# prime-slam/octreelib

Hardware: AMD Instinct MI355X
Metric: Mpoints/s insert+subdivide+RANSAC (higher is better)
Workload: dtype f64; 1 GPU; BASELINE config 3: Grid 1 m voxels, 10000000 planar points per GPU (scene 32x32x32 voxels), insert + subdivide(len>64) + map_leaf_points_cuda_ransac(H=1024, k=6, thr=0.01, poses_per_batch=10) incl. apply_mask; points_per_gpu=10000000, K=64, hypotheses=1024, leaves=575543

## Files before the change

### octreelib_amd/csrc/ransac.hip

```cpp
#include <algorithm>
#include <cstdlib>
#include <type_traits>

#include "forest.h"
#include "lookback.h"
#include "wave_utils.h"

namespace {

__device__ __forceinline__ double div_by_small_int(double c, int k) {
  const double kd = (double)k;
  const double zh = 1.0 / kd;
  const double zl = fma(-kd, zh, 1.0) / kd;
  const double a = fabs(c);
  if (!((int(a > 1e-290) | int(c == 0.0)) & int(a < 1e290))) return c / kd;
  return copysign(fma(c, zh, c * zl), c);
}

__device__ __forceinline__ bool coord_in_fast_range(double v) {
  const uint32_t hi = (uint32_t)__double2hiint(v), lo = (uint32_t)__double2loint(v);
  const uint32_t e = (hi >> 20) & 0x7FFu;
  return (e - (1023u - 30u)) <= 60u || (hi | lo) == 0u;
}

__device__ __forceinline__ void div3_by_small_int(double& cx, double& cy, double& cz, int k, bool fast = false) {
  const double kd = (double)k;
  const double zh = 1.0 / kd;
  const double zl = fma(-kd, zh, 1.0) / kd;
  if (fast) {
    cx = fma(cx, zh, cx * zl);
    cy = fma(cy, zh, cy * zl);
    cz = fma(cz, zh, cz * zl);
    return;
  }
  const double ax = fabs(cx), ay = fabs(cy), az = fabs(cz);
  const int ok = (int(ax > 1e-290) | int(cx == 0.0)) & int(ax < 1e290) &
                 (int(ay > 1e-290) | int(cy == 0.0)) & int(ay < 1e290) &
                 (int(az > 1e-290) | int(cz == 0.0)) & int(az < 1e290);
  if (!ok) {
    cx /= kd;
    cy /= kd;
    cz /= kd;
    return;
  }
  cx = copysign(fma(cx, zh, cx * zl), cx);
  cy = copysign(fma(cy, zh, cy * zl), cy);
  cz = copysign(fma(cz, zh, cz * zl), cz);
}

__device__ __forceinline__ double sqrt_rn_inrange(double s) {
  const double y = __builtin_amdgcn_rsq(s);
  double g = s * y;
  double h = y * 0.5;
  const double r = fma(-h, g, 0.5);
  g = fma(g, r, g);
  h = fma(h, r, h);
  double d = fma(-g, g, s);
  g = fma(d, h, g);
  d = fma(-g, g, s);
  return fma(d, h, g);
}
__device__ __forceinline__ double sqrt_rn_guarded(double s) {
  if (!(int(s >= 0x1p-700) & int(s < 0x1p1000))) return __dsqrt_rn(s);
  return sqrt_rn_inrange(s);
}

__device__ __forceinline__ void div3_by_norm_inrange(double& ax, double& ay, double& az, double norm) {
  double r = __builtin_amdgcn_rcp(norm);
  double e = fma(-norm, r, 1.0);
  r = fma(r, e, r);
  e = fma(-norm, r, 1.0);
  r = fma(r, e, r);
  const double qx = ax * r, qy = ay * r, qz = az * r;
  ax = copysign(fma(fma(-norm, qx, ax), r, qx), ax);
  ay = copysign(fma(fma(-norm, qy, ay), r, qy), ay);
  az = copysign(fma(fma(-norm, qz, az), r, qz), az);
}
__device__ __forceinline__ void div3_by_norm(double& ax, double& ay, double& az, double norm) {
  const double lo = 0x1p-400, hi = 0x1p500;
  const int ok = int(norm >= lo) & int(norm < hi) & (int(fabs(ax) >= lo) | int(ax == 0.0)) &
                 (int(fabs(ay) >= lo) | int(ay == 0.0)) & (int(fabs(az) >= lo) | int(az == 0.0));
  if (!ok) {
    ax /= norm;
    ay /= norm;
    az /= norm;
    return;
  }
  div3_by_norm_inrange(ax, ay, az, norm);
}

__device__ __forceinline__ void plane_from_moments(double cx, double cy, double cz, double xx, double xy,
                                                   double xz, double yy, double yz, double zz,
                                                   float (&plane)[4], bool fast = false) {
  const double det_x = yy * zz - yz * yz;
  const double det_y = xx * zz - xz * xz;
  const double det_z = xx * yy - xy * xy;
  const double cA = xz * yz - xy * zz;
  const double cB = xy * yz - xz * yy;
  const double cC = xy * xz - yz * xx;
  const bool is_x = det_x > det_y && det_x > det_z;
  const bool is_y = !is_x && det_y > det_z;
  double ax = is_x ? det_x : (is_y ? cA : cB);
  double ay = is_x ? cA : (is_y ? det_y : cC);
  double az = is_x ? cB : (is_y ? cC : det_z);
  const double s = ax * ax + ay * ay + az * az;
  if (fast && (uint32_t)__double2hiint(s) >= ((1023u - 400u) << 20)) {
    const double norm = sqrt_rn_inrange(s);
    div3_by_norm_inrange(ax, ay, az, norm);
  } else {
    const double norm = sqrt_rn_guarded(s);
    if (norm == 0.0) {
      plane[0] = plane[1] = plane[2] = plane[3] = 0.0f;
      return;
    }
    div3_by_norm(ax, ay, az, norm);
  }
  const double d = -(ax * cx + ay * cy + az * cz);
  plane[0] = (float)ax;
  plane[1] = (float)ay;
  plane[2] = (float)az;
  plane[3] = (float)d;
}

template <int KT, int KMAX>
__device__ __forceinline__ void plane_from_samples(const double (&sx)[KMAX],
                                                   const double (&sy)[KMAX],
                                                   const double (&sz)[KMAX], int k_rt,
                                                   float (&plane)[4], bool fast = false) {
  const int k = KT > 0 ? KT : k_rt;
  double cx = 0.0, cy = 0.0, cz = 0.0;
  if (fast) {
    cx = sx[0];
    cy = sy[0];
    cz = sz[0];
  } else {
    asm volatile("" ::: "memory");
    cx += sx[0];
    cy += sy[0];
    cz += sz[0];
  }
#pragma unroll
  for (int i = 1; i < (KT > 0 ? KT : KMAX); ++i) {
    if (i < k) {
      cx += sx[i];
      cy += sy[i];
      cz += sz[i];
    }
  }
  div3_by_small_int(cx, cy, cz, k, fast);
  double xx = 0.0, xy = 0.0, xz = 0.0, yy = 0.0, yz = 0.0, zz = 0.0;
#pragma unroll
  for (int i = 0; i < (KT > 0 ? KT : KMAX); ++i) {
    if (i < k) {
      const double rx = sx[i] - cx;
      const double ry = sy[i] - cy;
      const double rz = sz[i] - cz;
      if (i == 0) {
        xx = rx * rx;
// ... 56 lines not shown
  *risky = (x - (double)g0) > (1.0 - 0x1p-20);
  return g0 < n ? g0 : n;
}

__device__ __forceinline__ void plane_streamed(const double* __restrict__ hyp_row, int k, const BlockDesc& d,
                                               const double* __restrict__ xyz, float (&plane)[4]) {
  auto point = [&](int i) {
    const int g = sample_index_exact(hyp_row[i], d.n, d.vstart);
    return (g < d.n) ? (int64_t)d.pstart + g : (int64_t)d.pspill;
  };
  double cx = 0.0, cy = 0.0, cz = 0.0;
  for (int i = 0; i < k; ++i) {
    const int64_t p = point(i);
    cx += xyz[3 * p];
    cy += xyz[3 * p + 1];
    cz += xyz[3 * p + 2];
  }
  const double kd = (double)k;
  cx = cx / kd;
  cy = cy / kd;
  cz = cz / kd;
  double xx = 0.0, xy = 0.0, xz = 0.0, yy = 0.0, yz = 0.0, zz = 0.0;
  for (int i = 0; i < k; ++i) {
    const int64_t p = point(i);
    const double rx = xyz[3 * p] - cx, ry = xyz[3 * p + 1] - cy, rz = xyz[3 * p + 2] - cz;
    xx += rx * rx;
    xy += rx * ry;
    xz += rx * rz;
    yy += ry * ry;
    yz += ry * rz;
    zz += rz * rz;
  }
  plane_from_moments(cx, cy, cz, xx, xy, xz, yy, yz, zz, plane);
}

template <int THREADS, int HPL, int KT>
__device__ __forceinline__ void ransac_block_global(const BlockDesc& d, int be,
                                                    const double* __restrict__ xyz,
                                                    const double* __restrict__ hyp, int H, int k_rt,
                                                    double thr, const RansacOut& out,
                                                    unsigned long long* s_best, float* s_plane) {
  constexpr int KS = KT > 0 ? KT : RS_KMAX;
  const int k = KT > 0 ? KT : k_rt;
  const int n = d.n;
  const int64_t pstart = d.pstart;
  const double* __restrict__ pts = xyz + 3 * pstart;
  double pa[HPL], pb[HPL], pc[HPL], pd[HPL];
  int cnt[HPL];
#pragma unroll
  for (int q = 0; q < HPL; ++q) {
    const int t = threadIdx.x + q * THREADS;
    cnt[q] = -1;
    pa[q] = pb[q] = pc[q] = pd[q] = 0.0;
    if (t < H) {
      float pf[4];
      if constexpr (KT < 0) {
        plane_streamed(hyp + (int64_t)t * k, k, d, xyz, pf);
      } else {
        double sx[KS], sy[KS], sz[KS];
#pragma unroll
        for (int i = 0; i < KS; ++i) {
          sx[i] = sy[i] = sz[i] = 0.0;
          if (i < k) {
            const int g = sample_index_exact(hyp[(int64_t)t * k + i], n, d.vstart);
            const int64_t p = (g < n) ? pstart + g : (int64_t)d.pspill;
            sx[i] = xyz[3 * p];
            sy[i] = xyz[3 * p + 1];
            sz[i] = xyz[3 * p + 2];
          }
        }
        plane_from_samples<KT, KS>(sx, sy, sz, k, pf);
      }
      pa[q] = (double)pf[0];
      pb[q] = (double)pf[1];
      pc[q] = (double)pf[2];
      pd[q] = (double)pf[3];
      cnt[q] = 0;
    }
    __builtin_amdgcn_sched_barrier(0);
  }
  for (int i = 0; i < n; ++i) {
    const double x = pts[3 * (int64_t)i], y = pts[3 * (int64_t)i + 1], z = pts[3 * (int64_t)i + 2];
#pragma unroll
    for (int q = 0; q < HPL; ++q)
      cnt[q] += (plane_distance(pa[q], pb[q], pc[q], pd[q], x, y, z) < thr) ? 1 : 0;
  }
  unsigned long long best = 0;
#pragma unroll
  for (int q = 0; q < HPL; ++q) {
    const int t = threadIdx.x + q * THREADS;
    if (t < H) {
      const unsigned long long key =
          ((unsigned long long)(unsigned)cnt[q] << 32) | (unsigned)(0x7FFFFFFF - t);
      best = key > best ? key : best;
    }
  }
#pragma unroll
  for (int off = 32; off > 0; off >>= 1) {
    const unsigned long long o = __shfl_xor(best, off);
    best = o > best ? o : best;
  }
  if ((threadIdx.x & 63) == 0) s_best[threadIdx.x >> 6] = best;
  __syncthreads();
  best = s_best[0];
#pragma unroll
  for (int w = 1; w < THREADS / 64; ++w) best = s_best[w] > best ? s_best[w] : best;
  const int win = 0x7FFFFFFF - (int)(unsigned)(best & 0xFFFFFFFFu);
#pragma unroll
  for (int q = 0; q < HPL; ++q) {
    if ((int)threadIdx.x + q * THREADS == win) {
      const float f0 = (float)pa[q], f1 = (float)pb[q], f2 = (float)pc[q], f3 = (float)pd[q];
      s_plane[0] = f0; s_plane[1] = f1; s_plane[2] = f2; s_plane[3] = f3;
      if (out.plane) {
        out.plane[4 * (int64_t)be + 0] = f0; out.plane[4 * (int64_t)be + 1] = f1;
        out.plane[4 * (int64_t)be + 2] = f2; out.plane[4 * (int64_t)be + 3] = f3;
      }
      if (out.count) out.count[be] = cnt[q];
      if (out.index) out.index[be] = win;
    }
  }
  __syncthreads();
  const double a = (double)s_plane[0], bb = (double)s_plane[1], c = (double)s_plane[2],
               dd = (double)s_plane[3];
  for (int i = threadIdx.x; i < n; i += THREADS)
    out.mask[pstart + i] = (plane_distance(a, bb, c, dd, pts[3 * (int64_t)i], pts[3 * (int64_t)i + 1],
                                           pts[3 * (int64_t)i + 2]) < thr) ? 1 : 0;
}

typedef float f4 __attribute__((ext_vector_type(4)));
__device__ __forceinline__ float fma32(float a, float b, float c) { return __builtin_fmaf(a, b, c); }
__device__ __forceinline__ float min3abs(float m, float a, float b) {
  float r;
  asm("v_min3_f32 %0, %1, |%2|, |%3|" : "=v"(r) : "v"(m), "v"(a), "v"(b));
  return r;
}

template <int CTRL, int ROW_MASK>
__device__ __forceinline__ uint32_t dpp_u32(uint32_t v) {
  return (uint32_t)__builtin_amdgcn_update_dpp((int)v, (int)v, CTRL, ROW_MASK, 0xF, false);
}
__device__ __forceinline__ uint32_t wave_max_u32(uint32_t v) {
  v = max(v, dpp_u32<0xB1, 0xF>(v));
  v = max(v, dpp_u32<0x4E, 0xF>(v));
  v = max(v, dpp_u32<0x141, 0xF>(v));
  v = max(v, dpp_u32<0x140, 0xF>(v));
  v = max(v, dpp_u32<0x142, 0xA>(v));
  v = max(v, dpp_u32<0x143, 0xC>(v));
  return (uint32_t)__builtin_amdgcn_readlane((int)v, 63);
}
__device__ __forceinline__ float wave_max_nonneg_f32(float m) {
  return __uint_as_float(wave_max_u32(__float_as_uint(m)));
}

template <int THREADS>
__device__ __forceinline__ void stage_local(unsigned tx, double ox, double oy, double oz, const BlockDesc& d,
                                            double px, double py, double pz, f4* loc,
                                            float* wext, uint32_t* wfast, float* ext_out = nullptr,
                                            uint32_t* fast_out = nullptr) {
  float m = 0.f;
  if ((int)tx < d.n) {
    const float u = (float)(px - ox), v = (float)(py - oy), w = (float)(pz - oz);
    loc[tx] = f4{u, v, w, 0.f};
    m = fmaxf(fabsf(u), fmaxf(fabsf(v), fabsf(w)));
    if (!(m == m) || u != u || v != v || w != w) m = __int_as_float(0x7f800000);
  }
  m = wave_max_nonneg_f32(m);
  const bool inr = coord_in_fast_range(px) && coord_in_fast_range(py) && coord_in_fast_range(pz);
  const bool wave_fast = __all(inr);
  if (ext_out) {
    *ext_out = m;
    *fast_out = wave_fast ? 1u : 0u;
  } else if ((tx & 63) == 0) {
    wext[tx >> 6] = m;
    wfast[tx >> 6] = wave_fast ? 1u : 0u;
  }
}

template <int NH>
__device__ __forceinline__ void screen_group(const f4* __restrict__ loc, int n, const float* fa,
                                             const float* fb, const float* fc, const float* sto,
                                             float nthr2, int* cnt, float* margin) {
  float mg[2][NH];
#pragma unroll
  for (int h = 0; h < NH; ++h) mg[0][h] = mg[1][h] = __int_as_float(0x7f800000);
  for (int base = 0; base < n; base += 32) {
    const int m = __builtin_amdgcn_readfirstlane(min(32, n - base));
    uint32_t hist[NH];
#pragma unroll
    for (int h = 0; h < NH; ++h) hist[h] = 0;
    auto score = [&](const f4 L, float (&e)[NH]) {
#pragma unroll
      for (int h = 0; h < NH; ++h) {
        const float sv = fma32(fa[h], L.x, fma32(fb[h], L.y, fma32(fc[h], L.z, sto[h])));
        e[h] = fma32(sv, sv, nthr2);
        hist[h] = __builtin_amdgcn_alignbit(hist[h], __float_as_uint(e[h]), 31);
      }
    };
    int i = 0;
    for (; i + 4 <= m; i += 4) {
      const f4 L0 = loc[base + i], L1 = loc[base + i + 1], L2 = loc[base + i + 2],
               L3 = loc[base + i + 3];
      float e0[NH], e1[NH], e2[NH], e3[NH];
      score(L0, e0);
      score(L1, e1);
      score(L2, e2);
      score(L3, e3);
#pragma unroll
      for (int h = 0; h < NH; ++h) {
        mg[0][h] = min3abs(mg[0][h], e0[h], e1[h]);
        mg[1][h] = min3abs(mg[1][h], e2[h], e3[h]);
      }
    }
    for (; i < m; ++i) {
      float e[NH];
      score(loc[base + i], e);
#pragma unroll
      for (int h = 0; h < NH; ++h) mg[0][h] = min3abs(mg[0][h], e[h], e[h]);
    }
#pragma unroll
    for (int h = 0; h < NH; ++h) cnt[h] += __popc(hist[h]);
  }
#pragma unroll
  for (int h = 0; h < NH; ++h) margin[h] = fminf(mg[0][h], mg[1][h]);
}

struct PreConst {
  float qa, qb, qc;
  float e35;
  float thrblk;
};
__device__ __forceinline__ bool prescreen_constants(float extent, double ox, double oy, double oz, double thr,
                                                    PreConst& pc) {
  const float up = 0x1.004p0f;
  const float u = 0x1p-24f;
  const float E = extent;
  const float G = ((float)(fabs(ox) + fabs(oy) + fabs(oz)) + E) * 0x1.0002p0f;
  const float k1 = 16.f * (12.f * u + 0x1p-46f * (G / E) * 0x1.0002p0f) * 0x1.0002p0f;
  const float k0 = 16.f * (3.f * u * (E * E) + 0x1p-46f * G * E) * 0x1.0002p0f;
  pc.qa = (k1 + 0x1p-20f + k1 * k1 * 0x1p-4f) * up;
  pc.qb = (k0 + k1 * k0 * 0x1p-3f) * up;
  pc.qc = (k0 * k0 * 0x1p-4f) * up + 0x1p-98f;
  pc.e35 = 3.5f * E * up;
  const float eblk = (64.f * u * E + 0x1p-21f * G) * 0x1.0002p0f;
  const float thr_f = (float)thr * 0x1.0002p0f;
  pc.thrblk = (thr_f + eblk) * up;
  return E >= 0x1p-7f && E <= 0x1p7f && thr >= 0x1p-40 && thr <= 0x1p40 && eblk * 8.f <= thr_f;
}

template <int NH>
__device__ __forceinline__ void screen_ub(const f4* __restrict__ loc, int n, const float* fa, const float* fb,
                                          const float* fc, const float* sto, const float* T2, int* cnt) {
  for (int base = 0; base < n; base += 32) {
    const int m = __builtin_amdgcn_readfirstlane(min(32, n - base));
    uint32_t hist[NH];
#pragma unroll
    for (int h = 0; h < NH; ++h) hist[h] = 0;
    auto score = [&](const f4 L) {
#pragma unroll
      for (int h = 0; h < NH; ++h) {
        const float sv = fma32(fa[h], L.x, fma32(fb[h], L.y, fma32(fc[h], L.z, sto[h])));
        const float e = fma32(sv, sv, -T2[h]);
        hist[h] = __builtin_amdgcn_alignbit(hist[h], __float_as_uint(e), 31);
      }
    };
    int i = 0;
    for (; i + 4 <= m; i += 4) {
      const f4 L0 = loc[base + i], L1 = loc[base + i + 1], L2 = loc[base + i + 2], L3 = loc[base + i + 3];
      score(L0);
      score(L1);
      score(L2);
      score(L3);
    }
    for (; i < m; ++i) score(loc[base + i]);
#pragma unroll
    for (int h = 0; h < NH; ++h) cnt[h] += __popc(hist[h]);
  }
}

#ifdef RS_COUNTS
constexpr int RS_NSTAMPS = 24;
__device__ unsigned long long g_rs_stamps[RS_NSTAMPS];
#define RS_COUNT_INIT unsigned long long _rs_acc[RS_NSTAMPS] = {0, 0, 0, 0, 0, 0, 0, 0, 0, 0, 0, 0, 0, 0, 0, 0,  \
                                                                0, 0, 0, 0, 0, 0, 0, 0};                             \
                      const unsigned long long _rs_m0 = __builtin_amdgcn_s_memtime(),                      \
                                               _rs_r0 = __builtin_amdgcn_s_memrealtime()
#define RS_COUNT(k, v) _rs_acc[k] += (unsigned long long)(v)
#define RS_COUNT_FLUSH                                                                  \
  do {                                                                                  \
    if (threadIdx.x == 0) {                                                             \
      _rs_acc[0] = __builtin_amdgcn_s_memtime() - _rs_m0;                               \
      _rs_acc[1] = __builtin_amdgcn_s_memrealtime() - _rs_r0;                           \
      _rs_acc[10] += 1;                                                                 \
      for (int _k = 0; _k < RS_NSTAMPS; ++_k) atomicAdd(&g_rs_stamps[_k], _rs_acc[_k]); \
    }                                                                                   \
  } while (0)
#else
#define RS_COUNT_INIT do {} while (0)
#define RS_COUNT(k, v) do {} while (0)
#define RS_COUNT_FLUSH do {} while (0)
#endif

template <int THREADS, int HPL, int KT, bool FULLH, bool PT>
__global__ __launch_bounds__(THREADS, rs_minwaves(THREADS, KT)) void k_ransac(
    const double* __restrict__ xyz, const BlockDesc* __restrict__ sdesc,
    const uint32_t* __restrict__ lo_ptr, const uint32_t* __restrict__ hi_ptr, const double* __restrict__ hyp, int H,
    int k_rt, double thr, RansacOut out, const uint2* __restrict__ pos_tab, int no_prescreen) {
  static_assert(!PT || (KT > 0 && KT <= 6), "the position table packs up to six positions and their risk bits");
  static_assert(THREADS * HPL <= 1024, "hypothesis index in 10 bits");
  constexpr bool PRE = PT && KT >= 3 && HPL >= 2;
  constexpr int W = THREADS / 64;
  constexpr bool PARK = PRE && W == 1;
  constexpr int KS = KT > 0 ? KT : RS_KMAX;
  constexpr int GW = (KS + 3) / 4;
  constexpr int PRE_LIST = THREADS == 64 ? 512 : 256;
  constexpr bool OWN_LIST = PRE && W > 1;
  __shared__ uint16_t s_surv_all[OWN_LIST ? W : 1][OWN_LIST ? PRE_LIST : 1];
  uint16_t* const s_surv_own = s_surv_all[OWN_LIST ? (threadIdx.x >> 6) : 0];
  const int k = KT > 0 ? KT : k_rt;
  __shared__ double s_pts[3][3][THREADS];
  __shared__ uint32_t s_wbest[2][W];
  __shared__ float s_wplane[2][W][4];
  __shared__ f4 s_loc[3][THREADS];
  static_assert(!(PRE && W == 1) || PRE_LIST * sizeof(uint16_t) <= sizeof(s_loc[0]), "the survivor list fits an s_loc buffer");
  __shared__ float s_wext[3][W];
  __shared__ uint32_t s_wfast[3][W];
  const int lo = lo_ptr ? (int)*lo_ptr : 0;
  const int hi = (int)*hi_ptr;
  const int nbs = hi - lo;
  const int C = (nbs + (int)gridDim.x - 1) / (int)gridDim.x;
  int j = lo + (int)blockIdx.x * C;
  const int j_end = min(hi, j + C);
  if (j >= j_end) return;
  float ext_carry = 0.f;
  uint32_t fast_carry = 0;
  BlockDesc cur = sdesc[j];
  BlockDesc nxt = cur;
  if (j + 1 < j_end) nxt = sdesc[j + 1];
  {
    double px = 0.0, py = 0.0, pz = 0.0;
    if ((int)threadIdx.x <= cur.n) {
      const int64_t p = ((int)threadIdx.x < cur.n) ? (int64_t)cur.pstart + threadIdx.x : (int64_t)cur.pspill;
      px = xyz[3 * p];
      py = xyz[3 * p + 1];
      pz = xyz[3 * p + 2];
      s_pts[0][0][threadIdx.x] = px;
      s_pts[0][1][threadIdx.x] = py;
      s_pts[0][2][threadIdx.x] = pz;
    }
    stage_local<THREADS>(threadIdx.x, xyz[3 * (int64_t)cur.pstart], xyz[3 * (int64_t)cur.pstart + 1],
                         xyz[3 * (int64_t)cur.pstart + 2], cur, px, py, pz, s_loc[0], s_wext[0], s_wfast[0],
                         W == 1 ? &ext_carry : nullptr, W == 1 ? &fast_carry : nullptr);
  }
  __syncthreads();
  int buf = 0, par = 0;
  RS_COUNT_INIT;
  for (;;) {
    unsigned tx = threadIdx.x;
    asm volatile("" : "+v"(tx));
    const bool has_next = j + 1 < j_end;
    BlockDesc nxt2 = nxt;
    if (j + 2 < j_end) nxt2 = sdesc[j + 2];
    double rx = 0.0, ry = 0.0, rz = 0.0;
    auto pre_here = [&]() {
      unsigned t = tx;
      if constexpr (PARK) asm volatile("" : "+v"(t));
      return has_next && (int)t <= nxt.n;
    };
    const int nbuf = buf == 2 ? 0 : buf + 1;
    uint16_t* const s_surv = PARK ? (uint16_t*)&s_loc[nbuf][0] : s_surv_own;
    auto prefetch = [&]() {
      if (pre_here()) {
        const int64_t p = ((int)tx < nxt.n) ? (int64_t)nxt.pstart + tx : (int64_t)nxt.pspill;
        rx = xyz[3 * p];
        ry = xyz[3 * p + 1];
        rz = xyz[3 * p + 2];
      }
    };
    auto park = [&]() {
      if (pre_here()) {
        s_pts[nbuf][0][tx] = rx;
        s_pts[nbuf][1][tx] = ry;
        s_pts[nbuf][2][tx] = rz;
      }
    };
    double nox = 0.0, noy = 0.0, noz = 0.0;
    if constexpr (!PARK) {
      prefetch();
      if (has_next) {
        nox = xyz[3 * (int64_t)nxt.pstart];
        noy = xyz[3 * (int64_t)nxt.pstart + 1];
        noz = xyz[3 * (int64_t)nxt.pstart + 2];
      }
    }
    const int n = cur.n;
    const int be = (int)cur.pad[1];
    const double* __restrict__ lx = s_pts[buf][0];
    const double* __restrict__ ly = s_pts[buf][1];
    const double* __restrict__ lz = s_pts[buf][2];

    RS_COUNT(8, 1);
    RS_COUNT(11, n);
    float extent = W == 1 ? ext_carry : s_wext[buf][0];
#pragma unroll
    for (int w = 1; w < W; ++w) extent = fmaxf(extent, s_wext[buf][w]);
    uint32_t fastw = W == 1 ? fast_carry : s_wfast[buf][0];
#pragma unroll
    for (int w = 1; w < W; ++w) fastw &= s_wfast[buf][w];
    const bool blk_fast = __builtin_amdgcn_readfirstlane((int)fastw) != 0;
    const bool blk_sane = thr >= 0x1p-40 && thr <= 0x1p40 && extent < 0x1p60f;
    const bool fast_screen = blk_fast && thr >= 0x1p-40 && thr <= 0x1p40;
    const f4* __restrict__ loc = s_loc[buf];
    struct BlkConst {
      double ox, oy, oz;
      double delta_blk, dprime_thr, thr2;
      float nthr2;
      float delta_blk_f, thr2_f, dprime_thr_f;
    };
    auto blk_consts = [&]() {
      double th = thr;
      if constexpr (PARK) asm volatile("" : "+s"(th));
      BlkConst c;
      c.ox = lx[0]; c.oy = ly[0]; c.oz = lz[0];
      c.delta_blk = fma(0x1p-23 * 9.0, (double)extent,
                        0x1p-49 * (fabs(c.ox) + fabs(c.oy) + fabs(c.oz) + (double)extent + 1.0));
      c.dprime_thr = 0x1p-21 * (th * th);
      c.thr2 = th + th;
      c.nthr2 = -(float)(th * th);
      c.delta_blk_f = (float)c.delta_blk * 0x1.0002p0f;
      c.thr2_f = (float)(th + th) * 0x1.0002p0f;
      c.dprime_thr_f = (float)c.dprime_thr * 0x1.0002p0f;
      return c;
    };
    const BlkConst bc0 = blk_consts();
    auto consts_here = [&]() {
      if constexpr (PARK) return blk_consts();
      else return bc0;
    };
    const double ox = bc0.ox, oy = bc0.oy, oz = bc0.oz;

    uint32_t gpk[GW], rk = 0;
    float fa = 0.f, fb = 0.f, fc = 0.f, fd = 0.f, sto = 0.f, sdl = 0.f;
    int cnt = 0;
    auto load_pos = [&](const int t, const bool act) {
#pragma unroll
      for (int w = 0; w < GW; ++w) gpk[w] = 0;
      rk = 0;
      if constexpr (PT) {
        const uint2 e = pos_tab[(size_t)n * (size_t)H + (size_t)(act ? t : 0)];
        gpk[0] = e.x;
        if (GW > 1) gpk[GW - 1] = e.y & 0xFFFFu;
        rk = e.y >> 16;
      } else if (act) {
        const double* __restrict__ row = hyp + (int64_t)t * k;
#pragma unroll
        for (int i = 0; i < KS; ++i) {
          if (i < k) {
            bool risky;
            const int g = sample_index_cached(row[i], n, &risky);
            gpk[i >> 2] |= (uint32_t)g << (8 * (i & 3));
            rk |= (risky || g == n) ? (1u << i) : 0u;
          }
        }
      }
    };
    auto fit = [&](const int t, const bool act) {
      cnt = 0;
      fa = fb = fc = fd = sto = sdl = 0.f;
      if (FULLH || act) {
        const BlkConst bc = consts_here();
        const double ox = bc.ox, oy = bc.oy, oz = bc.oz, delta_blk = bc.delta_blk, dprime_thr = bc.dprime_thr;
        const float delta_blk_f = bc.delta_blk_f, thr2_f = bc.thr2_f, dprime_thr_f = bc.dprime_thr_f;
        double sx[KS], sy[KS], sz[KS];
        if (!__any(rk != 0u)) {
#pragma unroll
          for (int i = 0; i < KS; ++i) {
            sx[i] = sy[i] = sz[i] = 0.0;
            if (i < k) {
              const int g = (int)((gpk[i >> 2] >> (8 * (i & 3))) & 0xFFu);
              sx[i] = lx[g];
              sy[i] = ly[g];
              sz[i] = lz[g];
            }
          }
        } else {
#pragma unroll
          for (int i = 0; i < KS; ++i) {
            sx[i] = sy[i] = sz[i] = 0.0;
            if (i < k) {
              int g = (int)((gpk[i >> 2] >> (8 * (i & 3))) & 0xFFu);
              if (rk & (1u << i)) g = sample_index_exact(hyp[(int64_t)t * k + i], n, cur.vstart);
              sx[i] = lx[g];
              sy[i] = ly[g];
              sz[i] = lz[g];
            }
          }
        }
        float pf[4];
        plane_from_samples<KT, KS>(sx, sy, sz, k, pf, blk_fast);
        const double A = (double)pf[0], B = (double)pf[1], Cc = (double)pf[2], D = (double)pf[3];
        const double to = fma(A, ox, fma(B, oy, fma(Cc, oz, D)));
        fa = pf[0]; fb = pf[1]; fc = pf[2]; fd = pf[3];
        sto = (float)to;
        if (fast_screen) {
          const float dl = fma32(fabsf(sto), 0x1.0002p-21f, fma32(fabsf(pf[3]), 0x1.0002p-49f, delta_blk_f));
          sdl = fma32(dl, thr2_f + dl, dprime_thr_f) * 0x1.0002p0f;
        } else {
          const double delta = fma(0x1p-21, fabs(to), fma(0x1p-49, fabs(D), delta_blk));
          const double dprime = fma(delta, bc.thr2 + delta, dprime_thr) * 1.000001;
          const bool sane = blk_sane && (fabs(to) < 0x1p60);
          sdl = sane ? (float)dprime : __int_as_float(0x7f800000);
        }
      }
    };
    auto score = [&](const bool act) {
      float margin[1];
      int c1[1] = {0};
      RS_COUNT(14, 1);
      RS_COUNT(15, n);
      screen_group<1>(loc, n, &fa, &fb, &fc, &sto, consts_here().nthr2, c1, margin);
      cnt = c1[0];
      const bool redo = act && !(margin[0] > sdl);
      unsigned long long todo = __ballot(redo);
      RS_COUNT(13, __popcll(todo));
      while (todo) {
        const int src = __ffsll((long long)todo) - 1;
        todo &= todo - 1;
        const double A = (double)__uint_as_float(__builtin_amdgcn_readlane(__float_as_uint(fa), src));
        const double B = (double)__uint_as_float(__builtin_amdgcn_readlane(__float_as_uint(fb), src));
        const double Cc = (double)__uint_as_float(__builtin_amdgcn_readlane(__float_as_uint(fc), src));
        const double D = (double)__uint_as_float(__builtin_amdgcn_readlane(__float_as_uint(fd), src));
        int c = 0;
        for (int base = 0; base < n; base += 64) {
          const int ii = base + (int)(tx & 63u);
          const bool in = ii < n && plane_distance(A, B, Cc, D, lx[ii < n ? ii : 0], ly[ii < n ? ii : 0],
                                                   lz[ii < n ? ii : 0]) < thr;
          c += __popcll(__ballot(in));
        }
        if ((int)(tx & 63u) == src) cnt = c;
      }
    };
    uint32_t best = 0;
    float wa = 0.f, wb = 0.f, wc = 0.f, wd = 0.f;
    auto take = [&](const int t, const bool act) {
      if (act) {
        const uint32_t key = ((uint32_t)(cnt + 1) << 10) | (uint32_t)(1023 - t);
        if (key > best) {
          best = key;
          wa = fa; wb = fb; wc = fc; wd = fd;
        }
      }
    };
    {
      const int t = (int)tx;
      const bool act = FULLH || t < H;
      load_pos(t, act);
      fit(t, act);
      if constexpr (PARK) prefetch();
      score(act);
      take(t, act);
    }
    if constexpr (HPL > 1) {
      int Lcur = (int)wave_max_u32((FULLH || (int)tx < H) ? (uint32_t)cnt : 0u);
      if (Lcur != n) {
        int S = 0;
        bool use_list = false;
        if constexpr (PRE) {
          PreConst pc;
          const bool elig = prescreen_constants(extent, ox, oy, oz, thr, pc) && blk_fast && !no_prescreen;
          if (elig) {
            RS_COUNT(4, 1);
            constexpr bool TWO = THREADS == 64;
            typedef uint32_t __attribute__((may_alias)) u32a;
            const int budget = n - Lcur;
            int m1 = n, qhead = 0, qtail = 0;
            bool two_stage = false;
            f4* ploc = nullptr;
            u32a *qlo = nullptr, *qhi = nullptr;
            if constexpr (TWO) {
              m1 = min(n, (budget + RS_STAGE1_SLACK + 3) & ~3);
              two_stage = n - m1 >= RS_STAGE2_MIN;
              if (two_stage) {
                const int third = buf == 0 ? 2 : buf - 1;
                ploc = s_loc[third];
                qlo = (u32a*)&s_pts[third][0][0];
                qhi = (u32a*)&s_pts[buf == 2 ? 0 : buf + 1][0][0];
                static_assert(3 * RS_STAGE2_RING * sizeof(uint32_t) <= sizeof(s_pts[0]), "three words per idle buffer");
                const unsigned long long wl = __ballot(cnt == Lcur);
                const int src = __ffsll((long long)wl) - 1;
                const float A = __uint_as_float(__builtin_amdgcn_readlane(__float_as_uint(fa), src));
                const float B = __uint_as_float(__builtin_amdgcn_readlane(__float_as_uint(fb), src));
                const float Cc = __uint_as_float(__builtin_amdgcn_readlane(__float_as_uint(fc), src));
                const float To = __uint_as_float(__builtin_amdgcn_readlane(__float_as_uint(sto), src));
                const bool mine = (int)tx < n;
                const f4 Lp = loc[mine ? tx : 0];
                const float sv = fma32(A, Lp.x, fma32(B, Lp.y, fma32(Cc, Lp.z, To)));
                const bool far = mine && !(fma32(sv, sv, consts_here().nthr2) < 0.f);
                const unsigned long long mf = __ballot(far), mn = __ballot(mine && !far);
                const unsigned long long mm = far ? mf : mn;
                const int pos = (far ? 0 : __popcll(mf)) +
                                (int)__builtin_amdgcn_mbcnt_hi((uint32_t)(mm >> 32), __builtin_amdgcn_mbcnt_lo((uint32_t)mm, 0u));
                if (mine) ploc[pos] = Lp;
                __builtin_amdgcn_fence(__ATOMIC_ACQ_REL, "wavefront");
              } else {
                RS_COUNT(19, 1);
              }
            }
            auto survive = [&](const bool sv, const uint32_t ub, const int t) {
              const unsigned long long mk = __ballot(sv);
              if (sv) {
                const int pos = S + (int)__builtin_amdgcn_mbcnt_hi((uint32_t)(mk >> 32), __builtin_amdgcn_mbcnt_lo((uint32_t)mk, 0u));
                if (pos < PRE_LIST) s_surv[pos] = (uint16_t)((ub << 10) | (uint32_t)t);
              }
              S += __popcll(mk);
            };
            auto stage2 = [&](const int nq) {
              __builtin_amdgcn_fence(__ATOMIC_ACQ_REL, "wavefront");
              const bool mine = (int)tx < nq;
              const int e = (qhead + (mine ? (int)tx : 0)) & (RS_STAGE2_RING - 1);
              const float a = __uint_as_float(qlo[e]), b = __uint_as_float(qlo[RS_STAGE2_RING + e]),
                          c = __uint_as_float(qlo[2 * RS_STAGE2_RING + e]), to = __uint_as_float(qhi[e]),
                          T2 = __uint_as_float(qhi[RS_STAGE2_RING + e]);
              const uint32_t w = qhi[2 * RS_STAGE2_RING + e];
              int c2[1] = {(int)(w >> 10)};
              screen_ub<1>(ploc + m1, n - m1, &a, &b, &c, &to, &T2, c2);
              RS_COUNT(17, 64 * (n - m1));
              RS_COUNT(21, 1);
              survive(mine && c2[0] > Lcur, (uint32_t)c2[0], (int)(w & 1023u));
              qhead += nq;
            };
            auto prescreen = [&](auto nh_tag, const int qb) {
              constexpr int NH = decltype(nh_tag)::value;
              uint2 pe[NH];
              auto hyp_a = [&](const int h) { return (int)tx + (qb + h) * THREADS; };
#pragma unroll
              for (int h = 0; h < NH; ++h)
                pe[h] = pos_tab[(size_t)n * (size_t)H + (size_t)((FULLH || hyp_a(h) < H) ? hyp_a(h) : 0)];
              float qa[NH], qb_[NH], qc[NH], qto[NH], qT2[NH];
              bool qok[NH];
              int qcnt[NH];
              uint32_t risk = 0;
#pragma unroll
              for (int h = 0; h < NH; ++h) {
                const uint32_t w0 = pe[h].x, w1 = pe[h].y;
                f4 P[KS];
#pragma unroll
                for (int i = 0; i < KS; ++i) P[i] = loc[((i < 4 ? w0 : w1) >> (8 * (i & 3))) & 0xFFu];
                const float inv_k = 1.0f / (float)KS;
                float cx = P[0].x, cy = P[0].y, cz = P[0].z;
#pragma unroll
                for (int i = 1; i < KS; ++i) {
                  cx += P[i].x;
                  cy += P[i].y;
                  cz += P[i].z;
                }
                cx *= inv_k;
                cy *= inv_k;
                cz *= inv_k;
                float xx, xy, xz, yy, yz, zz;
                {
                  const float ax = P[0].x - cx, ay = P[0].y - cy, az = P[0].z - cz;
                  xx = ax * ax; xy = ax * ay; xz = ax * az; yy = ay * ay; yz = ay * az; zz = az * az;
                }
#pragma unroll
                for (int i = 1; i < KS; ++i) {
                  const float ax = P[i].x - cx, ay = P[i].y - cy, az = P[i].z - cz;
                  xx = fma32(ax, ax, xx); xy = fma32(ax, ay, xy); xz = fma32(ax, az, xz);
                  yy = fma32(ay, ay, yy); yz = fma32(ay, az, yz); zz = fma32(az, az, zz);
                }
                const float dx = fma32(yy, zz, -(yz * yz)), dy = fma32(xx, zz, -(xz * xz)), dz = fma32(xx, yy, -(xy * xy));
                const float cA = fma32(xz, yz, -(xy * zz)), cB = fma32(xy, yz, -(xz * yy)), cC = fma32(xy, xz, -(yz * xx));
                const bool is_x = dx > dy && dx > dz;
                const bool is_y = !is_x && dy > dz;
                const float m1 = is_x ? dx : (is_y ? cA : cB);
                const float m2 = is_x ? cA : (is_y ? dy : cC);
                const float m3 = is_x ? cB : (is_y ? cC : dz);
                const float ss = fma32(m3, m3, fma32(m2, m2, m1 * m1));
                const float r = __builtin_amdgcn_rsqf(ss);
                const float a = m1 * r, b = m2 * r, c = m3 * r;
                qa[h] = a; qb_[h] = b; qc[h] = c;
                float to = -fma32(c, cz, fma32(b, cy, a * cx));
                asm volatile("" : "+v"(to));
                qto[h] = to;
                const float T = (xx + yy) + zz;
                const float mu4 = fma32(fma32(pc.qa, T, pc.qb), T, pc.qc);
                const float gap = __builtin_fmaxf(__builtin_fmaxf(dx, dy), dz) - __builtin_amdgcn_fmed3f(dx, dy, dz);
                qok[h] = (ss * r > mu4) && (gap > mu4);
                risk |= w1;
                const float thr_h = fma32(pc.e35, mu4 * r, pc.thrblk);
                qT2[h] = thr_h * thr_h;
                qcnt[h] = 0;
              }
              if (__any((risk >> 16) != 0u)) {
#pragma unroll
                for (int h = 0; h < NH; ++h) qok[h] = qok[h] && (pe[h].y >> 16) == 0u;
              }
              RS_COUNT(12, NH);
              RS_COUNT(22, 64 * NH * n);
              if constexpr (TWO) {
                if (two_stage) {
                  bool bad = false;
#pragma unroll
                  for (int h = 0; h < NH; ++h) bad = bad || !qok[h];
                  if (__any(bad)) {
#pragma unroll
                    for (int h = 0; h < NH; ++h) {
                      if (!qok[h]) {
                        qa[h] = qb_[h] = qc[h] = qto[h] = 0.f;
                        qT2[h] = 1.f;
                      }
                    }
                  }
                  screen_ub<NH>(ploc, m1, qa, qb_, qc, qto, qT2, qcnt);
                  RS_COUNT(16, 64 * NH * m1);
#pragma unroll
                  for (int h = 0; h < NH; ++h) {
                    const bool alive = qcnt[h] > m1 - budget && (FULLH || hyp_a(h) < H);
                    const unsigned long long mk = __ballot(alive);
                    if (alive) {
                      const int e = (qtail + (int)__builtin_amdgcn_mbcnt_hi((uint32_t)(mk >> 32), __builtin_amdgcn_mbcnt_lo((uint32_t)mk, 0u))) &
                                    (RS_STAGE2_RING - 1);
                      qlo[e] = __float_as_uint(qa[h]);
                      qlo[RS_STAGE2_RING + e] = __float_as_uint(qb_[h]);
                      qlo[2 * RS_STAGE2_RING + e] = __float_as_uint(qc[h]);
                      qhi[e] = __float_as_uint(qto[h]);
                      qhi[RS_STAGE2_RING + e] = __float_as_uint(qT2[h]);
                      qhi[2 * RS_STAGE2_RING + e] = ((uint32_t)qcnt[h] << 10) | (uint32_t)hyp_a(h);
                    }
                    qtail += __popcll(mk);
                    RS_COUNT(18, __popcll(mk));
                    if (qtail - qhead >= 64) stage2(64);
                  }
                  return;
                }
              }
              screen_ub<NH>(loc, n, qa, qb_, qc, qto, qT2, qcnt);
              RS_COUNT(20, 64 * NH * n);
#pragma unroll
              for (int h = 0; h < NH; ++h)
                survive(!(qok[h] && qcnt[h] <= Lcur) && (FULLH || hyp_a(h) < H),
                        (THREADS == 64 && qok[h]) ? (uint32_t)qcnt[h] : 63u, hyp_a(h));
            };
            constexpr int PNH = 3;
            constexpr int TRIOS = (HPL - 1) / PNH, REST = (HPL - 1) % PNH;
#pragma unroll 1
            for (int i = 0; i < TRIOS; ++i) prescreen(std::integral_constant<int, PNH>{}, 1 + PNH * i);
            if constexpr (REST > 0) prescreen(std::integral_constant<int, (REST > 0 ? REST : 1)>{}, 1 + PNH * TRIOS);
            if constexpr (TWO) {
              if (qtail != qhead) stage2(qtail - qhead);
            }
            RS_COUNT(2, S);
            use_list = S <= PRE_LIST;
            if (!use_list) RS_COUNT(5, 1);
          }
          __builtin_amdgcn_fence(__ATOMIC_ACQ_REL, "wavefront");
        }
        if constexpr (PARK) park();
        const int nbatch = use_list ? ((S + 63) >> 6) : HPL - 1;
#pragma unroll 1
        for (int bt = 0; bt < nbatch; ++bt) {
          int t;
          bool act;
          if (use_list) {
            const int idx = bt * 64 + (int)(tx & 63u);
            const uint32_t ent = s_surv[idx < S ? idx : S - 1];
            t = (int)(ent & 1023u);
            act = idx < S && (THREADS != 64 || (int)(ent >> 10) > Lcur);
          } else {
            t = (int)tx + (bt + 1) * THREADS;
            act = FULLH || t < H;
          }
          if (!__any(act)) continue;
          RS_COUNT(3, 1);
          load_pos(t, act);
          fit(t, act);
          score(act);
          take(t, act);
          Lcur = max(Lcur, (int)wave_max_u32(act ? (uint32_t)cnt : 0u));
          if (Lcur == n) break;
        }
      } else {
        RS_COUNT(9, 1);
        if constexpr (PARK) park();
      }
    }
    const uint32_t wbest = wave_max_u32(best);
    float f0, f1, f2, f3;
    uint32_t gbest;
    if constexpr (W == 1) {
      const unsigned long long wl = __ballot(best == wbest && best != 0);
      const int src = wl ? __ffsll((long long)wl) - 1 : 0;
      gbest = wbest;
      f0 = __uint_as_float(__builtin_amdgcn_readlane(__float_as_uint(wa), src));
      f1 = __uint_as_float(__builtin_amdgcn_readlane(__float_as_uint(wb), src));
      f2 = __uint_as_float(__builtin_amdgcn_readlane(__float_as_uint(wc), src));
      f3 = __uint_as_float(__builtin_amdgcn_readlane(__float_as_uint(wd), src));
      if (!wl) f0 = f1 = f2 = f3 = 0.f;
    } else if (best == wbest && best != 0) {
      const int w = tx >> 6;
      s_wbest[par][w] = best;
      s_wplane[par][w][0] = wa;
      s_wplane[par][w][1] = wb;
      s_wplane[par][w][2] = wc;
      s_wplane[par][w][3] = wd;
    } else if (wbest == 0 && (tx & 63) == 0) {
      s_wbest[par][tx >> 6] = 0;
    }
    if constexpr (PARK) {
      __builtin_amdgcn_fence(__ATOMIC_ACQ_REL, "wavefront");
      if (pre_here()) {
        rx = s_pts[nbuf][0][tx];
        ry = s_pts[nbuf][1][tx];
        rz = s_pts[nbuf][2][tx];
      }
      if (has_next) {
        nox = s_pts[nbuf][0][0];
        noy = s_pts[nbuf][1][0];
        noz = s_pts[nbuf][2][0];
      }
    } else {
      park();
    }
    if (has_next)
      stage_local<THREADS>(tx, nox, noy, noz, nxt, rx, ry, rz, s_loc[nbuf], s_wext[nbuf], s_wfast[nbuf],
                           W == 1 ? &ext_carry : nullptr, W == 1 ? &fast_carry : nullptr);
    __syncthreads();
    if constexpr (W > 1) {
      gbest = s_wbest[par][0];
      int gw = 0;
#pragma unroll
      for (int w = 1; w < W; ++w) {
        if (s_wbest[par][w] > gbest) {
          gbest = s_wbest[par][w];
          gw = w;
        }
      }
      f0 = s_wplane[par][gw][0]; f1 = s_wplane[par][gw][1]; f2 = s_wplane[par][gw][2]; f3 = s_wplane[par][gw][3];
    }
    if (tx == 0) {
      if (out.plane) {
        out.plane[4 * (int64_t)be + 0] = f0; out.plane[4 * (int64_t)be + 1] = f1;
        out.plane[4 * (int64_t)be + 2] = f2; out.plane[4 * (int64_t)be + 3] = f3;
      }
      if (out.count) out.count[be] = (int32_t)(gbest >> 10) - 1;
      if (out.index) out.index[be] = 1023 - (int)(gbest & 1023u);
    }
    if ((int)tx < n) {
      const double dist = plane_distance((double)f0, (double)f1, (double)f2, (double)f3,
                                         lx[tx], ly[tx], lz[tx]);
      out.mask[(int64_t)cur.pstart + tx] = (dist < thr) ? 1 : 0;
    }
    if (!has_next) break;
    cur = nxt;
    nxt = nxt2;
    j += 1;
    buf = nbuf;
    par ^= 1;
  }
  RS_COUNT_FLUSH;
}

template <int THREADS, int HPL, int KT>
__device__ __forceinline__ void ransac_block_tiled(const BlockDesc& d, int be,
                                                   const double* __restrict__ xyz,
                                                   const double* __restrict__ hyp, int H, int k_rt,
                                                   double thr, const RansacOut& out, f4* s_loc,
                                                   float* s_wext, unsigned long long* s_best,
                                                   float* s_plane) {
  constexpr int KS = KT > 0 ? KT : RS_KMAX;
  constexpr int W = THREADS / 64;
  const int k = KT > 0 ? KT : k_rt;
  const int n = d.n;
  const int64_t pstart = d.pstart;
  const double* __restrict__ pts = xyz + 3 * pstart;
  const double ox = pts[0], oy = pts[1], oz = pts[2];
  float m = 0.f;
  for (int i = threadIdx.x; i < n; i += THREADS) {
    const float u = (float)(pts[3 * (int64_t)i] - ox), v = (float)(pts[3 * (int64_t)i + 1] - oy),
                w = (float)(pts[3 * (int64_t)i + 2] - oz);
    float mm = fmaxf(fabsf(u), fmaxf(fabsf(v), fabsf(w)));
    if (!(mm == mm) || u != u || v != v || w != w) mm = __int_as_float(0x7f800000);
    m = fmaxf(m, mm);
  }
#pragma unroll
  for (int off = 32; off > 0; off >>= 1) m = fmaxf(m, __shfl_xor(m, off));
  if ((threadIdx.x & 63) == 0) s_wext[threadIdx.x >> 6] = m;
  __syncthreads();
  float extent = s_wext[0];
#pragma unroll
  for (int w = 1; w < W; ++w) extent = fmaxf(extent, s_wext[w]);
  const double delta_blk = fma(0x1p-23 * 9.0, (double)extent,
                               0x1p-49 * (fabs(ox) + fabs(oy) + fabs(oz) + (double)extent + 1.0));
  const double dprime_thr = 0x1p-21 * (thr * thr);
  const bool blk_sane = thr >= 0x1p-40 && thr <= 0x1p40 && extent < 0x1p60f;
  const float nthr2 = -(float)(thr * thr);
  float fa[HPL], fb[HPL], fc[HPL], fd[HPL], sto[HPL], sdl[HPL], margin[HPL];
  int cnt[HPL];
#pragma unroll
  for (int q = 0; q < HPL; ++q) {
    const int t = threadIdx.x + q * THREADS;
    cnt[q] = 0;
    fa[q] = fb[q] = fc[q] = fd[q] = sto[q] = 0.f;
    sdl[q] = 0.f;
    margin[q] = __int_as_float(0x7f800000);
    if (t < H) {
      float pf[4];
      if constexpr (KT < 0) {
        plane_streamed(hyp + (int64_t)t * k, k, d, xyz, pf);
      } else {
        double sx[KS], sy[KS], sz[KS];
#pragma unroll
        for (int i = 0; i < KS; ++i) {
          sx[i] = sy[i] = sz[i] = 0.0;
          if (i < k) {
            const int g = sample_index_exact(hyp[(int64_t)t * k + i], n, d.vstart);
            const int64_t p = (g < n) ? pstart + g : (int64_t)d.pspill;
            sx[i] = xyz[3 * p];
            sy[i] = xyz[3 * p + 1];
            sz[i] = xyz[3 * p + 2];
          }
        }
        plane_from_samples<KT, KS>(sx, sy, sz, k, pf);
      }
      const double A = (double)pf[0], B = (double)pf[1], Cc = (double)pf[2], D = (double)pf[3];
      const double to = fma(A, ox, fma(B, oy, fma(Cc, oz, D)));
      const double delta = fma(0x1p-21, fabs(to), fma(0x1p-49, fabs(D), delta_blk));
      const double dprime = fma(delta, thr + thr + delta, dprime_thr) * 1.000001;
      const bool sane = blk_sane && (fabs(to) < 0x1p60);
      fa[q] = pf[0]; fb[q] = pf[1]; fc[q] = pf[2]; fd[q] = pf[3];
      sto[q] = (float)to;
      sdl[q] = sane ? (float)dprime : __int_as_float(0x7f800000);
    }
    __builtin_amdgcn_sched_barrier(0);
  }
  for (int t0 = 0; t0 < n; t0 += THREADS) {
    const int nt = min(THREADS, n - t0);
    if ((int)threadIdx.x < nt) {
      const int64_t i = t0 + threadIdx.x;
      s_loc[threadIdx.x] = f4{(float)(pts[3 * i] - ox), (float)(pts[3 * i + 1] - oy), (float)(pts[3 * i + 2] - oz), 0.f};
    }
    __syncthreads();
    float mt[HPL];
    screen_group<HPL>(s_loc, nt, fa, fb, fc, sto, nthr2, cnt, mt);
#pragma unroll
    for (int q = 0; q < HPL; ++q) margin[q] = fminf(margin[q], mt[q]);
    __syncthreads();
  }
#pragma unroll
  for (int q = 0; q < HPL; ++q) {
    const bool redo = (int)threadIdx.x + q * THREADS < H && !(margin[q] > sdl[q]);
    unsigned long long todo = __ballot(redo);
    while (todo) {
      const int src = __ffsll((long long)todo) - 1;
      todo &= todo - 1;
      const double A = (double)__uint_as_float(__builtin_amdgcn_readlane(__float_as_uint(fa[q]), src));
      const double B = (double)__uint_as_float(__builtin_amdgcn_readlane(__float_as_uint(fb[q]), src));
      const double Cc = (double)__uint_as_float(__builtin_amdgcn_readlane(__float_as_uint(fc[q]), src));
      const double D = (double)__uint_as_float(__builtin_amdgcn_readlane(__float_as_uint(fd[q]), src));
      int c = 0;
      for (int base = 0; base < n; base += 64) {
        const int ii = base + (int)(threadIdx.x & 63u);
        const int64_t jj = ii < n ? ii : 0;
        const bool in = ii < n && plane_distance(A, B, Cc, D, pts[3 * jj], pts[3 * jj + 1], pts[3 * jj + 2]) < thr;
        c += __popcll(__ballot(in));
      }
      if ((int)(threadIdx.x & 63u) == src) cnt[q] = c;
    }
  }
  unsigned long long best = 0;
#pragma unroll
  for (int q = 0; q < HPL; ++q) {
    const int t = threadIdx.x + q * THREADS;
    if (t < H) {
      const unsigned long long key = ((unsigned long long)(unsigned)cnt[q] << 32) | (unsigned)(0x7FFFFFFF - t);
      best = key > best ? key : best;
    }
  }
// ... 683 lines not shown
```

Measured before the change: 3933 Mpoints/s.

## Certify no-plane leaves via scatter eigen bound to skip RANSAC prescreen

When a leaf's inlier budget is one or two points, the wave computes f64 scatter sums with DPP reductions and uses a determinant/trace lower bound on the smallest eigenvalue to prove no plane can hold all (or all but one) points. Certified leaves skip the two-stage prescreen and only reject degenerate or risky hypotheses with a cheap cross-product check. The change also recomputes the lane id via mbcnt and makes the fast flag uniform through readfirstlane. It adds f64 wave reductions on small-budget leaves, and it depends on the bound being conservative so that results stay exact.

```diff
diff --git a/octreelib_amd/csrc/plane_cert.h b/octreelib_amd/csrc/plane_cert.h
--- /dev/null
+++ b/octreelib_amd/csrc/plane_cert.h
@@ -0,0 +1,61 @@
+#pragma once
+
+#if defined(__HIPCC__) || defined(__CUDACC__)
+#define PLANE_CERT_HD __host__ __device__ inline
+#else
+#define PLANE_CERT_HD inline
+#endif
+
+namespace plane_cert {
+
+struct Scatter {
+  double xx, xy, xz, yy, yz, zz;
+  double cx, cy, cz;
+  double tr;
+};
+
+PLANE_CERT_HD Scatter scatter_from_sums(int n, double sx, double sy, double sz, double sxx, double sxy, double sxz,
+                                        double syy, double syz, double szz) {
+  Scatter s;
+  const double inv_n = 1.0 / (double)n;
+  s.cx = sx * inv_n;
+  s.cy = sy * inv_n;
+  s.cz = sz * inv_n;
+  s.xx = sxx - sx * s.cx;
+  s.xy = sxy - sx * s.cy;
+  s.xz = sxz - sx * s.cz;
+  s.yy = syy - sy * s.cy;
+  s.yz = syz - sy * s.cz;
+  s.zz = szz - sz * s.cz;
+  s.tr = (s.xx + s.yy) + s.zz;
+  return s;
+}
+
+PLANE_CERT_HD bool eigen_floor_exceeds(double xx, double xy, double xz, double yy, double yz, double zz,
+                                       double tr_full, int m, double t) {
+  if (!(tr_full > 0x1p-200 && tr_full < 0x1p200 && t >= 0x1p-100 && t <= 0x1p100 && m >= 1)) return false;
+  const double tr = (xx + yy) + zz;
+  if (!(tr > 0.0)) return false;
+  const double det = (xx * (yy * zz - yz * yz) - xy * (xy * zz - yz * xz)) + xz * (xy * yz - yy * xz);
+  const double allowance = 0x1p-30 * ((tr_full * tr_full) * tr_full);
+  const double trb = tr + 0x1p-32 * tr_full;
+  const double lhs = 4.0 * (det - allowance);
+  const double rhs = ((double)m * (t * t)) * (1.0 + 0x1p-10) * (trb * trb);
+  return lhs > rhs;
+}
+
+PLANE_CERT_HD bool no_plane_holds_all(const Scatter& s, int n, double t) {
+  if (n < 3) return false;
+  return eigen_floor_exceeds(s.xx, s.xy, s.xz, s.yy, s.yz, s.zz, s.tr, n, t);
+}
+
+PLANE_CERT_HD bool no_plane_holds_others(const Scatter& s, int n, double rx, double ry, double rz, double t) {
+  if (n < 4) return false;
+  const double qx = rx - s.cx, qy = ry - s.cy, qz = rz - s.cz;
+  const double w = (double)n / (double)(n - 1);
+  const double wx = w * qx, wy = w * qy, wz = w * qz;
+  return eigen_floor_exceeds(s.xx - wx * qx, s.xy - wx * qy, s.xz - wx * qz, s.yy - wy * qy, s.yz - wy * qz,
+                             s.zz - wz * qz, s.tr, n - 1, t);
+}
+
+}
diff --git a/octreelib_amd/csrc/ransac.hip b/octreelib_amd/csrc/ransac.hip
--- a/octreelib_amd/csrc/ransac.hip
+++ b/octreelib_amd/csrc/ransac.hip
@@ -4,6 +4,7 @@
 
 #include "forest.h"
 #include "lookback.h"
+#include "plane_cert.h"
 #include "wave_utils.h"
 
 namespace {
@@ -366,7 +367,24 @@
   return __uint_as_float(wave_max_u32(__float_as_uint(m)));
 }
 
-template <int THREADS>
+template <int CTRL, int ROW_MASK>
+__device__ __forceinline__ double dpp_f64_or_zero(double v) {
+  const int lo = __builtin_amdgcn_update_dpp(0, __double2loint(v), CTRL, ROW_MASK, 0xF, false);
+  const int hi = __builtin_amdgcn_update_dpp(0, __double2hiint(v), CTRL, ROW_MASK, 0xF, false);
+  return __hiloint2double(hi, lo);
+}
+__device__ __forceinline__ double wave_sum_f64(double v) {
+  v += dpp_f64_or_zero<0xB1, 0xF>(v);
+  v += dpp_f64_or_zero<0x4E, 0xF>(v);
+  v += dpp_f64_or_zero<0x141, 0xF>(v);
+  v += dpp_f64_or_zero<0x140, 0xF>(v);
+  v += dpp_f64_or_zero<0x142, 0xA>(v);
+  v += dpp_f64_or_zero<0x143, 0xC>(v);
+  return __hiloint2double(__builtin_amdgcn_readlane(__double2hiint(v), 63),
+                          __builtin_amdgcn_readlane(__double2loint(v), 63));
+}
+
+template <int THREADS, bool SFAST = false>
 __device__ __forceinline__ void stage_local(unsigned tx, double ox, double oy, double oz, const BlockDesc& d,
                                             double px, double py, double pz, f4* loc,
                                             float* wext, uint32_t* wfast, float* ext_out = nullptr,
@@ -383,7 +401,7 @@
   const bool wave_fast = __all(inr);
   if (ext_out) {
     *ext_out = m;
-    *fast_out = wave_fast ? 1u : 0u;
+    *fast_out = SFAST ? (uint32_t)__builtin_amdgcn_readfirstlane(wave_fast ? 1 : 0) : (wave_fast ? 1u : 0u);
   } else if ((tx & 63) == 0) {
     wext[tx >> 6] = m;
     wfast[tx >> 6] = wave_fast ? 1u : 0u;
@@ -492,10 +510,10 @@
 }
 
 #ifdef RS_COUNTS
-constexpr int RS_NSTAMPS = 24;
+constexpr int RS_NSTAMPS = 32;
 __device__ unsigned long long g_rs_stamps[RS_NSTAMPS];
 #define RS_COUNT_INIT unsigned long long _rs_acc[RS_NSTAMPS] = {0, 0, 0, 0, 0, 0, 0, 0, 0, 0, 0, 0, 0, 0, 0, 0,  \
-                                                                0, 0, 0, 0, 0, 0, 0, 0};                             \
+                                                                0, 0, 0, 0, 0, 0, 0, 0, 0, 0, 0, 0, 0, 0, 0, 0};     \
                       const unsigned long long _rs_m0 = __builtin_amdgcn_s_memtime(),                      \
                                                _rs_r0 = __builtin_amdgcn_s_memrealtime()
 #define RS_COUNT(k, v) _rs_acc[k] += (unsigned long long)(v)
@@ -513,6 +531,7 @@
 #define RS_COUNT(k, v) do {} while (0)
 #define RS_COUNT_FLUSH do {} while (0)
 #endif
+
 
 template <int THREADS, int HPL, int KT, bool FULLH, bool PT>
 __global__ __launch_bounds__(THREADS, rs_minwaves(THREADS, KT)) void k_ransac(
@@ -561,7 +580,7 @@
       s_pts[0][1][threadIdx.x] = py;
       s_pts[0][2][threadIdx.x] = pz;
     }
-    stage_local<THREADS>(threadIdx.x, xyz[3 * (int64_t)cur.pstart], xyz[3 * (int64_t)cur.pstart + 1],
+    stage_local<THREADS, PARK>(threadIdx.x, xyz[3 * (int64_t)cur.pstart], xyz[3 * (int64_t)cur.pstart + 1],
                          xyz[3 * (int64_t)cur.pstart + 2], cur, px, py, pz, s_loc[0], s_wext[0], s_wfast[0],
                          W == 1 ? &ext_carry : nullptr, W == 1 ? &fast_carry : nullptr);
   }
@@ -570,6 +589,11 @@
   RS_COUNT_INIT;
   for (;;) {
     unsigned tx = threadIdx.x;
+    if constexpr (PARK) {
+      unsigned z = 0;
+      asm volatile("" : "+v"(z));
+      tx = __builtin_amdgcn_mbcnt_hi(~0u, __builtin_amdgcn_mbcnt_lo(~0u, z));
+    }
     asm volatile("" : "+v"(tx));
     const bool has_next = j + 1 < j_end;
     BlockDesc nxt2 = nxt;
@@ -786,13 +810,35 @@
             constexpr bool TWO = THREADS == 64;
             typedef uint32_t __attribute__((may_alias)) u32a;
             const int budget = n - Lcur;
+            bool certified = false;
+            if constexpr (TWO) {
+              if (budget <= 2) {
+                RS_COUNT(budget == 1 ? 24 : 25, 1);
+                const bool mine = (int)tx < n;
+                auto rel = [&](const double* __restrict__ l) { return l[mine ? tx : 0u] - l[0]; };
+                double sum[9];
+#pragma unroll
+                for (int q = 0; q < 9; ++q) {
+                  const double* __restrict__ la = q < 3 ? (q == 0 ? lx : q == 1 ? ly : lz) : (q < 6 ? lx : q < 8 ? ly : lz);
+                  const double* __restrict__ lb = (q == 3) ? lx : (q == 4 || q == 6) ? ly : lz;
+                  sum[q] = wave_sum_f64(q < 3 ? rel(la) : rel(la) * rel(lb));
+                  __builtin_amdgcn_sched_barrier(0);
+                }
+                const plane_cert::Scatter sc = plane_cert::scatter_from_sums(n, sum[0], sum[1], sum[2], sum[3], sum[4],
+                                                                             sum[5], sum[6], sum[7], sum[8]);
+                const double t = (double)pc.thrblk;
+                if (budget == 1) certified = plane_cert::no_plane_holds_all(sc, n, t);
+                else certified = __all(!mine || plane_cert::no_plane_holds_others(sc, n, rel(lx), rel(ly), rel(lz), t));
+                if (certified) RS_COUNT(budget == 1 ? 26 : 27, 1);
+              }
+            }
             int m1 = n, qhead = 0, qtail = 0;
             bool two_stage = false;
             f4* ploc = nullptr;
             u32a *qlo = nullptr, *qhi = nullptr;
             if constexpr (TWO) {
               m1 = min(n, (budget + RS_STAGE1_SLACK + 3) & ~3);
-              two_stage = n - m1 >= RS_STAGE2_MIN;
+              two_stage = !certified && n - m1 >= RS_STAGE2_MIN;
               if (two_stage) {
                 const int third = buf == 0 ? 2 : buf - 1;
                 ploc = s_loc[third];
@@ -815,7 +861,7 @@
                                 (int)__builtin_amdgcn_mbcnt_hi((uint32_t)(mm >> 32), __builtin_amdgcn_mbcnt_lo((uint32_t)mm, 0u));
                 if (mine) ploc[pos] = Lp;
                 __builtin_amdgcn_fence(__ATOMIC_ACQ_REL, "wavefront");
-              } else {
+              } else if (!certified) {
                 RS_COUNT(19, 1);
               }
             }
@@ -956,9 +1002,39 @@
             };
             constexpr int PNH = 3;
             constexpr int TRIOS = (HPL - 1) / PNH, REST = (HPL - 1) % PNH;
+            if (TWO && certified) {
+              const float E = extent;
+              const float G = ((float)(fabs(lx[0]) + fabs(ly[0]) + fabs(lz[0])) + E) * 0x1.0002p0f;
+              const float E2 = E * E;
+              const float floor2 = fma32(0x1p-74f * (G * G), E2, 0x1p-24f * (E2 * E2)) * 0x1.0002p0f;
 #pragma unroll 1
-            for (int i = 0; i < TRIOS; ++i) prescreen(std::integral_constant<int, PNH>{}, 1 + PNH * i);
-            if constexpr (REST > 0) prescreen(std::integral_constant<int, (REST > 0 ? REST : 1)>{}, 1 + PNH * TRIOS);
+              for (int g = 1; g < HPL; ++g) {
+                const int t = (int)tx + g * THREADS;
+                const bool real = FULLH || t < H;
+                const uint2 e = pos_tab[(size_t)n * (size_t)H + (size_t)(real ? t : 0)];
+                uint32_t p[KS];
+#pragma unroll
+                for (int i = 0; i < KS; ++i) p[i] = ((i < 4 ? e.x : e.y) >> (8 * (i & 3))) & 0xFFu;
+                uint32_t p1 = p[KS - 1], p2 = p[KS - 1];
+#pragma unroll
+                for (int i = KS - 2; i >= 1; --i) p1 = p[i] != p[0] ? p[i] : p1;
+#pragma unroll
+                for (int i = KS - 2; i >= 2; --i) p2 = (p[i] != p[0] && p[i] != p1) ? p[i] : p2;
+                const bool risky = (e.y >> 16) != 0u;
+                const f4 P0 = loc[risky ? 0u : p[0]], P1 = loc[risky ? 0u : p1], P2 = loc[risky ? 0u : p2];
+                const float ux = P1.x - P0.x, uy = P1.y - P0.y, uz = P1.z - P0.z;
+                const float vx = P2.x - P0.x, vy = P2.y - P0.y, vz = P2.z - P0.z;
+                const float cx = fma32(uy, vz, -(uz * vy)), cy = fma32(uz, vx, -(ux * vz)), cz = fma32(ux, vy, -(uy * vx));
+                const float c2 = fma32(cz, cz, fma32(cy, cy, cx * cx));
+                const bool vouched = !risky && c2 > floor2;
+                RS_COUNT(28, __popcll(__ballot(real && !vouched)));
+                survive(real && !vouched, 63u, t);
+              }
+            } else {
+#pragma unroll 1
+              for (int i = 0; i < TRIOS; ++i) prescreen(std::integral_constant<int, PNH>{}, 1 + PNH * i);
+              if constexpr (REST > 0) prescreen(std::integral_constant<int, (REST > 0 ? REST : 1)>{}, 1 + PNH * TRIOS);
+            }
             if constexpr (TWO) {
               if (qtail != qhead) stage2(qtail - qhead);
             }
@@ -1035,7 +1111,7 @@
       park();
     }
     if (has_next)
-      stage_local<THREADS>(tx, nox, noy, noz, nxt, rx, ry, rz, s_loc[nbuf], s_wext[nbuf], s_wfast[nbuf],
+      stage_local<THREADS, PARK>(tx, nox, noy, noz, nxt, rx, ry, rz, s_loc[nbuf], s_wext[nbuf], s_wfast[nbuf],
                            W == 1 ? &ext_carry : nullptr, W == 1 ? &fast_carry : nullptr);
     __syncthreads();
     if constexpr (W > 1) {
```

Result: faster. 3997 Mpoints/s, median of 6 (+1.6%).
